# pengsongyou/openscene

Hardware: AMD Instinct MI355X
Metric: active voxels/sec MinkUNet18A fwd+bwd @2cm ScanNet; per-point query ms (higher is better)
Workload: dtype f32 (bf16x6 split-precision MFMA, fp32 accumulate); 1 GPU; ScanNet distillation step (configs[2]): MinkUNet18A, 768-d head, 1 synthetic S100k scene/GPU (100999 voxels on rank 0, 2 cm), training-mode BN; timed = coordinate+kernel maps, forward, cosine loss, backward, gradient all-reduce, Adam step; arch=MinkUNet18A, feature_dim=768, voxels_rank0=100999, parallelism=dp1

## Files before the change

include/openscene_amd.h:

```cpp
#ifndef OPENSCENE_AMD_H
#define OPENSCENE_AMD_H

#include <stddef.h>
#include <stdint.h>

#ifdef __cplusplus
extern "C" {
#endif

#define OSN_OK 0
#define OSN_E_ARG (-1)
#define OSN_E_HIP (-2)
#define OSN_E_WS (-3)
#define OSN_E_RANGE (-4)

typedef void* osn_stream_t;

int osn_version(void);
const char* osn_last_error(void);
int osn_device_ok(void);

int64_t osn_hash_capacity(int64_t n);
size_t osn_coords_unique_ws_bytes(int64_t n);

// ... 138 lines not shown
                         const float* residual, int relu, float momentum, float* mean, float* var,
                         float* running_mean, float* running_var, float* y, void* ws, size_t ws_bytes,
                         osn_stream_t stream);
int osn_bn_backward(const float* x, const float* y, const float* gy, const float* mean,
                    const float* var, const float* gamma, float eps, int relu, int training,
                    float* gx, float* gres, float* ggamma, float* gbeta,
                    int64_t n, int c, void* ws, size_t ws_bytes, osn_stream_t stream);

int osn_bn_apply2(const float* x, const float* mean, const float* var, const float* gamma,
                  const float* beta, float eps, const float* residual, int relu, float* y,
                  float* y2, int64_t ld2, int64_t n, int c, osn_stream_t stream);
int osn_bn_forward_train2(const float* x, int64_t n, int c, const float* gamma, const float* beta, float eps,
                          const float* residual, int relu, float momentum, float* mean, float* var,
                          float* running_mean, float* running_var, float* y, float* y2, int64_t ld2,
                          void* ws, size_t ws_bytes, osn_stream_t stream);
int osn_bn_backward_multi(const float* x, const float* y, const float* const* gy_host, const int64_t* gy_ld_host,
                          int n_gy, const float* mean, const float* var, const float* gamma, float eps, int relu,
                          int training, float* gx, float* gres, float* ggamma, float* gbeta,
                          int64_t n, int c, void* ws, size_t ws_bytes, osn_stream_t stream);
int osn_bn_backward_multi2(const float* x, const float* y, const float* const* gy_host, const int64_t* gy_ld_host, int n_gy,
                           const float* mean, const float* var, const float* gamma, const float* beta, float eps, int relu,
                           int training, float* gx, float* gres, float* ggamma, float* gbeta, int64_t n, int c, void* ws,
                           size_t ws_bytes, osn_stream_t stream);

size_t osn_distill_loss_state_bytes(int64_t n, int64_t n_sel);
int osn_distill_loss_fwd(const float* out, const int64_t* sel, const float* target, int64_t n, int64_t n_sel, int d, int kind,
                         float* loss, void* state, size_t state_bytes, osn_stream_t stream);
int osn_distill_loss_bwd(const float* out, const float* target, const float* gloss, int64_t n, int64_t n_sel, int d, int kind,
                         float* gout, const void* state, size_t state_bytes, osn_stream_t stream);
int osn_distill_loss_bwd_rows(const float* out, const float* target, const float* gloss, int64_t n, int64_t n_sel, int d, int kind,
                              float* gout, float* grows, const void* state, size_t state_bytes, osn_stream_t stream);
int osn_distill_loss_check(const void* state, int64_t n, int64_t n_sel, osn_stream_t stream);

int osn_adam_step(float* params, const float* grads, float* exp_avg, float* exp_avg_sq, int64_t n, int64_t step, float lr,
                  float beta1, float beta2, float eps, float weight_decay, osn_stream_t stream);

int osn_sgd_step(float* params, const float* grads, float* momentum_buf, int64_t n, float lr, float momentum, float dampening,
                 float weight_decay, int nesterov, int first, osn_stream_t stream);

size_t osn_seg_loss_state_bytes(int64_t n_lab, int c);
int osn_seg_loss_fwd(const float* logits, const int64_t* rows, const int64_t* labels, int64_t n, int64_t n_lab, int c,
                     int64_t ignore_index, float* loss, int64_t* pred, int64_t* confusion, void* state, size_t state_bytes,
                     osn_stream_t stream);
int osn_seg_loss_bwd(const float* logits, const int64_t* labels, const float* gloss, int64_t n, int c, int64_t ignore_index,
                     float* glogits, const void* state, size_t state_bytes, osn_stream_t stream);
int osn_seg_loss_check(const void* state, int64_t n, int64_t n_lab, int c, osn_stream_t stream);
// ... 267 lines not shown
```

openscene_amd/_lib.py:

```python
import ctypes
import os
import threading

_HERE = os.path.dirname(os.path.abspath(__file__))
LIB_PATH = os.environ.get("OSN_LIB_PATH") or os.path.join(_HERE, "lib", "libopenscene_amd.so")

_c = ctypes
_vp, _i32, _i64, _sz, _f32 = _c.c_void_p, _c.c_int, _c.c_int64, _c.c_size_t, _c.c_float

PROTOTYPES = {
    "osn_version": (_i32, []),
    "osn_last_error": (_c.c_char_p, []),
    "osn_device_ok": (_i32, []),
    "osn_hash_capacity": (_i64, [_i64]),
    "osn_coords_unique_ws_bytes": (_sz, [_i64]),
    "osn_coords_unique": (_i32, [_vp, _i64, _i32, _vp, _vp, _i64, _vp, _vp, _vp, _c.POINTER(_i64), _vp, _sz, _vp]),
    "osn_coords_unique_async": (_i32, [_vp, _i64, _vp, _i32, _vp, _vp, _i64, _vp, _vp, _vp, _vp, _vp, _vp, _sz, _vp]),
    "osn_coords_pyramid_async": (_i32, [_vp, _i64, _vp, _i32, _vp, _vp, _i64, _vp, _vp, _vp, _vp, _vp, _sz, _vp]),
    "osn_kmap_build": (_i32, [_vp, _vp, _i64, _vp, _i64, _i32, _i32, _vp, _vp, _vp]),
    "osn_kmap_build_self": (_i32, [_vp, _vp, _i64, _vp, _i64, _i32, _i32, _vp, _vp, _vp]),
    "osn_kmap_transpose": (_i32, [_vp, _i64, _i32, _i64, _vp, _vp]),
    "osn_kmap_sort_ws_bytes": (_sz, [_i64]),
    "osn_kmap_sort": (_i32, [_vp, _i64, _i32, _vp, _vp, _vp, _vp, _vp, _sz, _vp]),
    "osn_kmap_count": (_i32, [_vp, _i64, _i32, _vp, _vp]),
# ... 44 lines not shown
    "osn_seg_loss_fwd": (_i32, [_vp, _vp, _vp, _i64, _i64, _i32, _i64, _vp, _vp, _vp, _vp, _sz, _vp]),
    "osn_seg_loss_bwd": (_i32, [_vp, _vp, _vp, _i64, _i32, _i64, _vp, _vp, _sz, _vp]),
    "osn_seg_loss_check": (_i32, [_vp, _i64, _i64, _i32, _vp]),
    "osn_seg_vote": (_i32, [_vp, _vp, _i64, _i64, _i32, _vp, _vp]),
    "osn_spconv_fwd_ws_ws_bytes": (_sz, [_i64, _i32, _i32, _i32]),
    "osn_spconv_fwd_ws": (_i32, [_vp, _i64, _vp, _vp, _i64, _i32, _i32, _vp, _vp, _i64, _i32, _i32, _i32, _vp, _sz, _vp]),
    "osn_spconv_wgrad_tl_partial": (_i32, [_vp, _vp, _vp, _i32, _vp, _i64, _i64, _i32, _i32, _i32, _vp, _sz, _vp, _vp]),
    "osn_wgrad_tl_reduce_batch": (_i32, [_vp, _i32, _vp]),
    "osn_stem_conv_fwd": (_i32, [_vp, _vp, _vp, _vp, _i64, _i32, _i32, _i32, _vp]),
    "osn_bn_ws_bytes": (_sz, [_i64, _i32]),
    "osn_bn_stats": (_i32, [_vp, _i64, _i32, _vp, _vp, _vp, _vp, _f32, _vp, _sz, _vp]),
    "osn_bn_apply": (_i32, [_vp, _vp, _vp, _vp, _vp, _f32, _vp, _i32, _vp, _i64, _i32, _vp]),
    "osn_bn_forward_train": (_i32, [_vp, _i64, _i32, _vp, _vp, _f32, _vp, _i32, _f32, _vp, _vp, _vp, _vp, _vp, _vp, _sz, _vp]),
    "osn_bn_backward": (_i32, [_vp, _vp, _vp, _vp, _vp, _vp, _f32, _i32, _i32, _vp, _vp, _vp, _vp, _i64, _i32,
                               _vp, _sz, _vp]),
    "osn_bn_apply2": (_i32, [_vp, _vp, _vp, _vp, _vp, _f32, _vp, _i32, _vp, _vp, _i64, _i64, _i32, _vp]),
    "osn_spconv_fwd_rg_ok": (_i32, [_i64, _i32, _i32, _i32]),
    "osn_spconv_fwd_rg": (_i32, [_vp, _i64, _vp, _vp, _vp, _vp, _i64, _i32, _i32, _i32, _vp]),
    "osn_bn_forward_train2": (_i32, [_vp, _i64, _i32, _vp, _vp, _f32, _vp, _i32, _f32, _vp, _vp, _vp, _vp, _vp, _vp, _i64, _vp, _sz, _vp]),
    "osn_bn_backward_multi": (_i32, [_vp, _vp, _vp, _vp, _i32, _vp, _vp, _vp, _f32, _i32, _i32, _vp, _vp, _vp, _vp, _i64, _i32,
                                     _vp, _sz, _vp]),
    "osn_bn_backward_multi2": (_i32, [_vp, _vp, _vp, _vp, _i32, _vp, _vp, _vp, _vp, _f32, _i32, _i32, _vp, _vp, _vp, _vp, _i64, _i32,
                                     _vp, _sz, _vp]),
    "osn_net_plan_query": (_i32, [_vp, _vp, _i32, _vp]),
    "osn_net_forward": (_i32, [_vp, _vp, _vp]),
    "osn_net_backward": (_i32, [_vp, _vp, _vp]),
    "osn_maps_build": (_i32, [_vp, _i32, _vp, _i32, _vp, _vp, _vp, _i32, _vp]),
    "osn_events_create": (_vp, [_i32]),
    "osn_events_destroy": (None, [_vp]),
    "osn_prof_create": (_vp, [_i32]),
    "osn_prof_destroy": (None, [_vp]),
    "osn_prof_filter": (_i32, [_vp, _vp, _i32]),
    "osn_prof_read": (_i32, [_vp, _vp, _vp, _i32, _i32]),
    "osn_relu_fwd": (_i32, [_vp, _vp, _i64, _vp]),
    "osn_relu_bwd": (_i32, [_vp, _vp, _vp, _i64, _vp]),
    "osn_add": (_i32, [_vp, _vp, _vp, _i64, _vp]),
    "osn_cat2": (_i32, [_vp, _i32, _vp, _i32, _vp, _i64, _vp]),
    "osn_cat2_bwd": (_i32, [_vp, _vp, _i32, _vp, _i32, _i64, _vp]),
    "osn_cosine_query": (_i32, [_vp, _vp, _vp, _vp, _vp, _i64, _i32, _i32, _vp]),
    "osn_query_ensemble_ws_bytes": (_sz, [_i64]),
    "osn_query_ensemble": (_i32, [_vp, _vp, _vp, _vp, _vp, _vp, _vp, _vp, _i64, _i32, _i32, _vp, _sz, _vp]),
    "osn_cosine_query_vote": (_i32, [_vp, _vp, _vp, _vp, _vp, _i64, _i32, _i32, _vp]),
    "osn_query_ensemble_vote": (_i32, [_vp, _vp, _vp, _vp, _vp, _vp, _vp, _vp, _i64, _i32, _i32, _vp, _sz, _vp]),
    "osn_eval_confusion": (_i32, [_vp, _vp, _i64, _i32, _vp, _vp, _i64, _vp, _i32, _vp, _vp, _i32, _vp]),
    "osn_eval_check": (_i32, [_vp, _vp]),
    "osn_bank_append": (_i32, [_vp, _i64, _vp, _i64, _i32, _vp, _i64, _vp, _vp]),
# ... 99 lines not shown
```

openscene_amd/csrc/bn.hip:

```cpp
#include "common.h"
#include "epilogue.h"

namespace osn {

constexpr int CR_COLS = 64;
constexpr int CR_RL = 16;
constexpr int CR_MAX_BLOCKS = 512;

constexpr int BN_MAX_SRC = 3;
struct GySrc {
    const float* p[BN_MAX_SRC];
    int64_t ld[BN_MAX_SRC];
    int n;
};

__device__ inline float4 gy_load(const GySrc& s, int64_t r, int col) {
    float4 g = *reinterpret_cast<const float4*>(s.p[0] + r * s.ld[0] + col);
#pragma unroll
    for (int i = 1; i < BN_MAX_SRC; ++i)
        if (i < s.n) {
            const float4 v = *reinterpret_cast<const float4*>(s.p[i] + r * s.ld[i] + col);
            g.x += v.x; g.y += v.y; g.z += v.z; g.w += v.w;
        }
    return g;
}


struct ColReducePlan {
    int n_rb;
    int n_cg;
    int rows_per_block;
};

static ColReducePlan plan_colreduce(int64_t n, int c) {
    ColReducePlan p;
    p.n_cg = int(cdiv(c, CR_COLS));
    int64_t rb = cdiv(n, 4 * CR_RL);
    if (rb > CR_MAX_BLOCKS) rb = CR_MAX_BLOCKS;
    if (rb < 1) rb = 1;
    p.rows_per_block = int(cdiv(cdiv(n, rb), CR_RL) * CR_RL);
    p.n_rb = int(cdiv(n, p.rows_per_block));
    if (p.n_rb < 1) p.n_rb = 1;
    return p;
}

template <int MODE, bool STORE_G>
__device__ __forceinline__ void col_reduce_body(const float* __restrict__ x, const float* __restrict__ y, const GySrc gy,
                                                const float* __restrict__ mean, const float* __restrict__ var, float eps,
                                                int relu, int64_t n, int c, int rows_per_block, double* __restrict__ partial,
                                                const float* __restrict__ gamma, const float* __restrict__ beta,
                                                float* __restrict__ gres) {
    static_assert(!STORE_G || MODE == 1, "only the backward sums form g");
    __shared__ double red[2][CR_RL][CR_COLS];
    const int tid = threadIdx.x;
    const int cl = tid & 15, rl = tid >> 4;
    const int col = blockIdx.y * CR_COLS + cl * 4;
    const bool on = col < c;
    const int64_t r0 = int64_t(blockIdx.x) * rows_per_block;
    const int64_t r1 = min(n, r0 + rows_per_block);
    double s1[4] = {0, 0, 0, 0}, s2[4] = {0, 0, 0, 0};
    float4 mu = make_float4(0, 0, 0, 0), is = make_float4(0, 0, 0, 0);
    float4 ga = make_float4(0, 0, 0, 0), be = make_float4(0, 0, 0, 0);
    const bool from_x = MODE == 1 && !STORE_G && relu && !y;
    if (MODE == 1 && on) {
        mu = *reinterpret_cast<const float4*>(mean + col);
        const float4 v = *reinterpret_cast<const float4*>(var + col);
        is = make_float4(bn_is(v.x, eps), bn_is(v.y, eps), bn_is(v.z, eps), bn_is(v.w, eps));
        if (from_x) {
            ga = *reinterpret_cast<const float4*>(gamma + col);
            be = *reinterpret_cast<const float4*>(beta + col);
        }
    }
    if (on) {
        for (int64_t r = r0 + rl; r < r1; r += CR_RL) {
            const float4 xv = *reinterpret_cast<const float4*>(x + r * c + col);
            if (MODE == 0) {
                s1[0] += xv.x; s1[1] += xv.y; s1[2] += xv.z; s1[3] += xv.w;
                s2[0] += double(xv.x) * xv.x; s2[1] += double(xv.y) * xv.y;
                s2[2] += double(xv.z) * xv.z; s2[3] += double(xv.w) * xv.w;
            } else {
                float4 g = gy_load(gy, r, col);
                if (from_x) {
                    g.x = bn_val(xv.x, mu.x, is.x, ga.x, be.x) > 0.f ? g.x : 0.f;
                    g.y = bn_val(xv.y, mu.y, is.y, ga.y, be.y) > 0.f ? g.y : 0.f;
                    g.z = bn_val(xv.z, mu.z, is.z, ga.z, be.z) > 0.f ? g.z : 0.f;
                    g.w = bn_val(xv.w, mu.w, is.w, ga.w, be.w) > 0.f ? g.w : 0.f;
                } else if (relu) {
                    const float4 yv = *reinterpret_cast<const float4*>(y + r * c + col);
                    g.x = yv.x > 0.f ? g.x : 0.f; g.y = yv.y > 0.f ? g.y : 0.f;
                    g.z = yv.z > 0.f ? g.z : 0.f; g.w = yv.w > 0.f ? g.w : 0.f;
                }
                if (STORE_G) *reinterpret_cast<float4*>(gres + r * c + col) = g;
                s1[0] += g.x; s1[1] += g.y; s1[2] += g.z; s1[3] += g.w;
                s2[0] += double(g.x) * ((xv.x - mu.x) * is.x); s2[1] += double(g.y) * ((xv.y - mu.y) * is.y);
                s2[2] += double(g.z) * ((xv.z - mu.z) * is.z); s2[3] += double(g.w) * ((xv.w - mu.w) * is.w);
            }
        }
    }
#pragma unroll
    for (int j = 0; j < 4; ++j) {
        red[0][rl][cl * 4 + j] = s1[j];
        red[1][rl][cl * 4 + j] = s2[j];
    }
    __syncthreads();
    if (tid < 2 * CR_COLS) {
        const int which = tid / CR_COLS, cc = tid % CR_COLS;
        double s = 0;
#pragma unroll
        for (int r = 0; r < CR_RL; ++r) s += red[which][r][cc];
        const int gc = blockIdx.y * CR_COLS + cc;
        if (gc < c) partial[(int64_t(blockIdx.x) * 2 + which) * c + gc] = s;
    }
}

template <int MODE>
__global__ __launch_bounds__(256) void col_reduce_kernel(const float* __restrict__ x, const float* __restrict__ y,
                                                         const GySrc gy, const float* __restrict__ mean,
                                                         const float* __restrict__ var, float eps, int relu, int64_t n,
                                                         int c, int rows_per_block, double* __restrict__ partial,
                                                         const float* __restrict__ gamma, const float* __restrict__ beta) {
    col_reduce_body<MODE, false>(x, y, gy, mean, var, eps, relu, n, c, rows_per_block, partial, gamma, beta, nullptr);
}

__global__ __launch_bounds__(256) void col_reduce_gres_kernel(const float* __restrict__ x, const float* __restrict__ y,
                                                              const GySrc gy, const float* __restrict__ mean,
                                                              const float* __restrict__ var, float eps, int relu, int64_t n,
                                                              int c, int rows_per_block, double* __restrict__ partial,
                                                              float* __restrict__ gres) {
    col_reduce_body<1, true>(x, y, gy, mean, var, eps, relu, n, c, rows_per_block, partial, nullptr, nullptr, gres);
}

constexpr int FIN_COLS = 16, FIN_PARTS = 64;

constexpr int FIN_ITERS = CR_MAX_BLOCKS / FIN_PARTS;

__device__ inline void finalize_sums(const double* __restrict__ partial, int n_rb, int c, double& s1, double& s2,
                                     int& col) {
    __shared__ double red[2][FIN_PARTS][FIN_COLS];
    const int cl = threadIdx.x & (FIN_COLS - 1), part = threadIdx.x / FIN_COLS;
    col = blockIdx.x * FIN_COLS + cl;
    double va[FIN_ITERS], vb[FIN_ITERS];
    const int cc = col < c ? col : 0;
#pragma unroll
    for (int i = 0; i < FIN_ITERS; ++i) {
        const int blk = part + FIN_PARTS * i;
        const int bc = blk < n_rb ? blk : 0;
        va[i] = partial[(int64_t(bc) * 2 + 0) * c + cc];
        vb[i] = partial[(int64_t(bc) * 2 + 1) * c + cc];
    }
    double a = 0, b = 0;
#pragma unroll
    for (int i = 0; i < FIN_ITERS; ++i) {
// ... 33 lines not shown
    double v = s2 / double(n) - m * m;
    if (v < 0) v = 0;
    mean[j] = float(m);
    var[j] = float(v);
    if (running_mean) running_mean[j] = (1.f - momentum) * running_mean[j] + momentum * float(m);
    if (running_var) {
        const double unb = n > 1 ? v * double(n) / double(n - 1) : v;
        running_var[j] = (1.f - momentum) * running_var[j] + momentum * float(unb);
    }
}

__global__ __launch_bounds__(FIN_COLS * FIN_PARTS) void bn_bwd_finalize_kernel(const double* __restrict__ partial,
                                                                              int n_rb, int c,
                                                                              float* __restrict__ sum_g,
                                                                              float* __restrict__ sum_gx) {
    double s1, s2;
    int j;
    finalize_sums(partial, n_rb, c, s1, s2, j);
    if (threadIdx.x >= FIN_COLS || j >= c) return;
    sum_g[j] = float(s1);
    sum_gx[j] = float(s2);
}

__device__ inline float4 ld4(const float* p) { return *reinterpret_cast<const float4*>(p); }


__global__ __launch_bounds__(256) void bn_apply_kernel(const float* __restrict__ x, const float* __restrict__ mean,
                                                       const float* __restrict__ var, const float* __restrict__ gamma,
                                                       const float* __restrict__ beta, float eps,
                                                       const float* __restrict__ residual, int relu,
                                                       float* __restrict__ y, float* __restrict__ y2, int64_t ld2,
                                                       int64_t total4, int c4) {
    for (int64_t e = int64_t(blockIdx.x) * blockDim.x + threadIdx.x; e < total4; e += int64_t(gridDim.x) * blockDim.x) {
        const int col = int(e % c4) * 4;
        const float4 xv = ld4(x + e * 4), mu = ld4(mean + col), vv = ld4(var + col), ga = ld4(gamma + col),
                     be = ld4(beta + col);
        float4 o;
        o.x = bn_val(xv.x, mu.x, bn_is(vv.x, eps), ga.x, be.x);
        o.y = bn_val(xv.y, mu.y, bn_is(vv.y, eps), ga.y, be.y);
        o.z = bn_val(xv.z, mu.z, bn_is(vv.z, eps), ga.z, be.z);
        o.w = bn_val(xv.w, mu.w, bn_is(vv.w, eps), ga.w, be.w);
        if (residual) {
            const float4 rv = ld4(residual + e * 4);
            o.x += rv.x; o.y += rv.y; o.z += rv.z; o.w += rv.w;
        }
        if (relu) {
            o.x = bn_relu(o.x); o.y = bn_relu(o.y); o.z = bn_relu(o.z); o.w = bn_relu(o.w);
        }
        *reinterpret_cast<float4*>(y + e * 4) = o;
        if (y2) *reinterpret_cast<float4*>(y2 + (e / c4) * ld2 + col) = o;
    }
}

template <bool LOAD_G>
__device__ __forceinline__ void bn_bwd_apply_body(const float* __restrict__ x, const float* __restrict__ y, const GySrc& gy,
                                                  const float* __restrict__ mean, const float* __restrict__ var,
                                                  const float* __restrict__ gamma, float eps, int relu, int training,
                                                  const float* __restrict__ sum_g, const float* __restrict__ sum_gx, float inv_n,
                                                  float* __restrict__ gx, float* __restrict__ gres, int64_t total4, int c4,
                                                  const float* __restrict__ beta) {
    const bool from_x = !LOAD_G && relu && !y;
    for (int64_t e = int64_t(blockIdx.x) * blockDim.x + threadIdx.x; e < total4; e += int64_t(gridDim.x) * blockDim.x) {
        const int col = int(e % c4) * 4;
        float4 g = LOAD_G ? ld4(gres + e * 4) : gy_load(gy, e / c4, col);
        const float4 vv = ld4(var + col), ga = ld4(gamma + col);
        const float4 is = make_float4(bn_is(vv.x, eps), bn_is(vv.y, eps), bn_is(vv.z, eps), bn_is(vv.w, eps));
        float4 xv = make_float4(0, 0, 0, 0), mu = make_float4(0, 0, 0, 0);
        if (training || from_x) { xv = ld4(x + e * 4); mu = ld4(mean + col); }
        if (LOAD_G) {
        } else if (from_x) {
            const float4 be = ld4(beta + col);
            g.x = bn_val(xv.x, mu.x, is.x, ga.x, be.x) > 0.f ? g.x : 0.f;
            g.y = bn_val(xv.y, mu.y, is.y, ga.y, be.y) > 0.f ? g.y : 0.f;
            g.z = bn_val(xv.z, mu.z, is.z, ga.z, be.z) > 0.f ? g.z : 0.f;
            g.w = bn_val(xv.w, mu.w, is.w, ga.w, be.w) > 0.f ? g.w : 0.f;
        } else if (relu) {
            const float4 yv = ld4(y + e * 4);
            g.x = yv.x > 0.f ? g.x : 0.f; g.y = yv.y > 0.f ? g.y : 0.f;
            g.z = yv.z > 0.f ? g.z : 0.f; g.w = yv.w > 0.f ? g.w : 0.f;
        }
        if (!LOAD_G && gres) *reinterpret_cast<float4*>(gres + e * 4) = g;
        float4 o;
        if (training) {
            const float4 sg = ld4(sum_g + col), sx = ld4(sum_gx + col);
            o.x = ga.x * is.x * (g.x - sg.x * inv_n - (xv.x - mu.x) * is.x * sx.x * inv_n);
            o.y = ga.y * is.y * (g.y - sg.y * inv_n - (xv.y - mu.y) * is.y * sx.y * inv_n);
            o.z = ga.z * is.z * (g.z - sg.z * inv_n - (xv.z - mu.z) * is.z * sx.z * inv_n);
            o.w = ga.w * is.w * (g.w - sg.w * inv_n - (xv.w - mu.w) * is.w * sx.w * inv_n);
        } else {
            o.x = ga.x * is.x * g.x; o.y = ga.y * is.y * g.y; o.z = ga.z * is.z * g.z; o.w = ga.w * is.w * g.w;
        }
        *reinterpret_cast<float4*>(gx + e * 4) = o;
    }
}

__global__ __launch_bounds__(256) void bn_bwd_apply_kernel(const float* __restrict__ x, const float* __restrict__ y,
                                                           const GySrc gy, const float* __restrict__ mean,
                                                           const float* __restrict__ var, const float* __restrict__ gamma,
                                                           float eps, int relu, int training,
                                                           const float* __restrict__ sum_g,
                                                           const float* __restrict__ sum_gx, float inv_n,
                                                           float* __restrict__ gx, float* __restrict__ gres,
                                                           int64_t total4, int c4, const float* __restrict__ beta) {
    bn_bwd_apply_body<false>(x, y, gy, mean, var, gamma, eps, relu, training, sum_g, sum_gx, inv_n, gx, gres, total4, c4, beta);
}

__global__ __launch_bounds__(256) void bn_bwd_apply_gres_kernel(const float* __restrict__ x, const float* __restrict__ mean,
                                                                const float* __restrict__ var, const float* __restrict__ gamma,
                                                                float eps, int training, const float* __restrict__ sum_g,
                                                                const float* __restrict__ sum_gx, float inv_n,
                                                                float* __restrict__ gx, const float* __restrict__ gres,
                                                                int64_t total4, int c4) {
    bn_bwd_apply_body<true>(x, nullptr, GySrc{}, mean, var, gamma, eps, 0, training, sum_g, sum_gx, inv_n, gx,
                            const_cast<float*>(gres), total4, c4, nullptr);
}

constexpr int SB_THREADS = 1024, SB_RL = 512, SB_PER = 8, SB_COLS = 8;
constexpr int SB_MAX_ROWS = SB_RL * SB_PER;
// ... 86 lines not shown
            const float4 rv = ld4(residual + int64_t(r) * c + col);
            o.x += rv.x; o.y += rv.y; o.z += rv.z; o.w += rv.w;
        }
        if (relu) {
            o.x = bn_relu(o.x); o.y = bn_relu(o.y); o.z = bn_relu(o.z); o.w = bn_relu(o.w);
        }
        *reinterpret_cast<float4*>(y + int64_t(r) * c + col) = o;
        if (y2) *reinterpret_cast<float4*>(y2 + int64_t(r) * ld2 + col) = o;
    }
}

static bool ranges_overlap(const float* a, size_t na, const float* b, size_t nb) {
    const uintptr_t a0 = reinterpret_cast<uintptr_t>(a), b0 = reinterpret_cast<uintptr_t>(b);
    return a0 < b0 + nb * sizeof(float) && b0 < a0 + na * sizeof(float);
}

static int ew_grid(int64_t total4) {
    int64_t g = cdiv(total4, 256);
    if (g > 2048) g = 2048;
    if (g < 1) g = 1;
    return int(g);
}

}

using namespace osn;

extern "C" size_t osn_bn_ws_bytes(int64_t n, int c) {
    (void)n;
    return size_t(CR_MAX_BLOCKS) * 2 * size_t(c) * 8 + 256;
}

extern "C" int osn_bn_stats(const float* x, int64_t n, int c, float* mean, float* var, float* running_mean,
                            float* running_var, float momentum, void* ws, size_t ws_bytes, osn_stream_t stream) {
    hipStream_t st = static_cast<hipStream_t>(stream);
    OSN_REQUIRE(n >= 1 && c >= 4 && (c & 3) == 0, OSN_E_ARG, "osn_bn_stats: need n >= 1 and c %% 4 == 0 (n=%lld c=%d)", (long long)n, c);
    OSN_REQUIRE(x && mean && var && aligned16(x), OSN_E_ARG, "osn_bn_stats: null or unaligned pointer");
    ColReducePlan p = plan_colreduce(n, c);
    const size_t need = size_t(p.n_rb) * 2 * size_t(c) * 8;
    OSN_REQUIRE(ws && ws_bytes >= need, OSN_E_WS, "osn_bn_stats: workspace %zu < %zu", ws_bytes, need);
    double* partial = static_cast<double*>(ws);
    hipLaunchKernelGGL((col_reduce_kernel<0>), dim3(p.n_rb, p.n_cg), dim3(256), 0, st, x, (const float*)nullptr,
                       GySrc{}, (const float*)nullptr, (const float*)nullptr, 0.f, 0, n, c,
                       p.rows_per_block, partial, (const float*)nullptr, (const float*)nullptr);
    hipLaunchKernelGGL(bn_stats_finalize_kernel, dim3(cdiv(c, FIN_COLS)), dim3(FIN_COLS * FIN_PARTS), 0, st, partial, p.n_rb, n, c, mean, var,
                       running_mean, running_var, momentum);
    OSN_LAUNCH_CHECK();
    return OSN_OK;
}

extern "C" int osn_bn_apply2(const float* x, const float* mean, const float* var, const float* gamma, const float* beta,
                             float eps, const float* residual, int relu, float* y, float* y2, int64_t ld2, int64_t n, int c,
                             osn_stream_t stream) {
    hipStream_t st = static_cast<hipStream_t>(stream);
    OSN_REQUIRE(n >= 0 && c >= 4 && (c & 3) == 0, OSN_E_ARG, "osn_bn_apply: need c %% 4 == 0 (c=%d)", c);
    if (n == 0) return OSN_OK;
    OSN_REQUIRE(x && mean && var && gamma && beta && y, OSN_E_ARG, "osn_bn_apply: null pointer");
    OSN_REQUIRE(aligned16(x) && aligned16(y) && aligned16(mean) && aligned16(var) && aligned16(gamma) && aligned16(beta) &&
                    (!residual || aligned16(residual)),
                OSN_E_ARG, "osn_bn_apply: pointers must be 16-byte aligned");
    OSN_REQUIRE(!y2 || (aligned16(y2) && ld2 >= c && (ld2 & 3) == 0), OSN_E_ARG,
                "osn_bn_apply2: the second destination needs a 16-byte aligned pointer and a row stride >= c, %% 4 == 0");
    const int64_t total4 = n * (c / 4);
    hipLaunchKernelGGL(bn_apply_kernel, dim3(ew_grid(total4)), dim3(256), 0, st, x, mean, var, gamma, beta, eps,
                       residual, relu, y, y2, ld2, total4, c / 4);
    OSN_LAUNCH_CHECK();
    return OSN_OK;
}

extern "C" int osn_bn_apply(const float* x, const float* mean, const float* var, const float* gamma, const float* beta,
                            float eps, const float* residual, int relu, float* y, int64_t n, int c,
                            osn_stream_t stream) {
    return osn_bn_apply2(x, mean, var, gamma, beta, eps, residual, relu, y, nullptr, 0, n, c, stream);
}

extern "C" int osn_bn_forward_train2(const float* x, int64_t n, int c, const float* gamma, const float* beta, float eps,
                                     const float* residual, int relu, float momentum, float* mean, float* var,
                                     float* running_mean, float* running_var, float* y, float* y2, int64_t ld2, void* ws,
                                     size_t ws_bytes, osn_stream_t stream) {
    if (n >= 1 && n <= SB_MAX_ROWS && c >= 4 && (c & 3) == 0) {
        hipStream_t st = static_cast<hipStream_t>(stream);
        OSN_REQUIRE(x && mean && var && gamma && beta && y, OSN_E_ARG, "osn_bn_forward_train: null pointer");
        OSN_REQUIRE(aligned16(x) && aligned16(y) && aligned16(gamma) && aligned16(beta) && (!residual || aligned16(residual)),
                    OSN_E_ARG, "osn_bn_forward_train: pointers must be 16-byte aligned");
        OSN_REQUIRE(!y2 || (aligned16(y2) && ld2 >= c && (ld2 & 3) == 0), OSN_E_ARG,
                    "osn_bn_forward_train2: the second destination needs a 16-byte aligned pointer and a row stride >= c, %% 4 == 0");
        hipLaunchKernelGGL(bn_small_fwd_kernel, dim3(unsigned(cdiv(c, SB_COLS))), dim3(SB_THREADS), 0, st, x, int(n), c, gamma,
// ... 28 lines not shown
    OSN_REQUIRE(!beta || aligned16(beta), OSN_E_ARG, "osn_bn_backward: beta must be 16-byte aligned");
    OSN_REQUIRE(aligned16(x) && aligned16(gx) && aligned16(mean) && aligned16(var) && aligned16(gamma) &&
                    aligned16(ggamma) && aligned16(gbeta) && (!y || aligned16(y)) && (!gres || aligned16(gres)),
                OSN_E_ARG, "osn_bn_backward: pointers must be 16-byte aligned");
    GySrc src{};
    src.n = n_gy;
    for (int i = 0; i < BN_MAX_SRC; ++i) {
        const int j = i < n_gy ? i : 0;
        OSN_REQUIRE(gy[j] && aligned16(gy[j]) && gy_ld[j] >= c && (gy_ld[j] & 3) == 0, OSN_E_ARG,
                    "osn_bn_backward: gradient source %d needs a 16-byte aligned pointer and a row stride >= c, %% 4 == 0", j);
        src.p[i] = gy[j];
        src.ld[i] = gy_ld[j];
    }
    ColReducePlan p = plan_colreduce(n, c);
    const size_t need = size_t(p.n_rb) * 2 * size_t(c) * 8;
    OSN_REQUIRE(ws && ws_bytes >= need, OSN_E_WS, "osn_bn_backward: workspace %zu < %zu", ws_bytes, need);
    double* partial = static_cast<double*>(ws);
    const size_t span = size_t(n) * size_t(c);
    bool via_gres = gres != nullptr && !ranges_overlap(gres, span, x, span) && !(y && ranges_overlap(gres, span, y, span)) &&
                    !ranges_overlap(gres, span, gx, span);
    for (int i = 0; via_gres && i < n_gy; ++i)
        via_gres = !ranges_overlap(gres, span, src.p[i], size_t(n - 1) * size_t(src.ld[i]) + size_t(c));
    const dim3 rgrid(p.n_rb, p.n_cg);
    if (via_gres)
        hipLaunchKernelGGL(col_reduce_gres_kernel, rgrid, dim3(256), 0, st, x, y, src, mean, var, eps, relu, n, c,
                           p.rows_per_block, partial, gres);
    else
        hipLaunchKernelGGL((col_reduce_kernel<1>), rgrid, dim3(256), 0, st, x, y, src, mean, var, eps, relu, n, c,
                           p.rows_per_block, partial, gamma, beta);
    hipLaunchKernelGGL(bn_bwd_finalize_kernel, dim3(cdiv(c, FIN_COLS)), dim3(FIN_COLS * FIN_PARTS), 0, st, partial, p.n_rb, c, gbeta, ggamma);
    const int64_t total4 = n * (c / 4);
    if (via_gres)
        hipLaunchKernelGGL(bn_bwd_apply_gres_kernel, dim3(ew_grid(total4)), dim3(256), 0, st, x, mean, var, gamma, eps, training,
                           gbeta, ggamma, 1.f / float(n), gx, (const float*)gres, total4, c / 4);
    else
        hipLaunchKernelGGL(bn_bwd_apply_kernel, dim3(ew_grid(total4)), dim3(256), 0, st, x, y, src, mean, var, gamma, eps,
                           relu, training, gbeta, ggamma, 1.f / float(n), gx, gres, total4, c / 4, beta);
    OSN_LAUNCH_CHECK();
    return OSN_OK;
}

extern "C" int osn_bn_backward_multi(const float* x, const float* y, const float* const* gy, const int64_t* gy_ld, int n_gy,
                                     const float* mean, const float* var, const float* gamma, float eps, int relu,
                                     int training, float* gx, float* gres, float* ggamma, float* gbeta, int64_t n, int c,
                                     void* ws, size_t ws_bytes, osn_stream_t stream) {
    OSN_REQUIRE(!relu || y, OSN_E_ARG, "osn_bn_backward_multi: relu needs y (or osn_bn_backward_multi2 with beta)");
    return osn_bn_backward_multi2(x, y, gy, gy_ld, n_gy, mean, var, gamma, nullptr, eps, relu, training, gx, gres, ggamma, gbeta, n, c,
                                  ws, ws_bytes, stream);
}

extern "C" int osn_bn_backward(const float* x, const float* y, const float* gy, const float* mean, const float* var,
                               const float* gamma, float eps, int relu, int training, float* gx, float* gres,
                               float* ggamma, float* gbeta, int64_t n, int c, void* ws, size_t ws_bytes,
                               osn_stream_t stream) {
    const int64_t ld = c;
    return osn_bn_backward_multi(x, y, &gy, &ld, 1, mean, var, gamma, eps, relu, training, gx, gres, ggamma, gbeta, n, c, ws,
                                 ws_bytes, stream);
}
```

openscene_amd/ops.py:

```python
import ctypes
import os
import threading
import weakref

import torch

from . import _lib
from ._lib import check

_vp = ctypes.c_void_p

_profiler = None


def set_profiler(p):
    global _profiler
    _profiler = p


_raw_stream_of = torch._C._cuda_getCurrentRawStream
_current_device = torch._C._cuda_getDevice


def _prof_start(kind, dev, **meta):
# ... 922 lines not shown
def bn_backward_multi(x, y, gys, mean, var, gamma, eps, relu, training, want_gres, beta=None, gres_out=None):
    dev = x.device
    lib = _prep(dev)
    n, c = x.shape
    if relu and y is None and (beta is None or want_gres):
        raise ValueError("batch-norm backward with ReLU needs y, or beta and no residual")
    views = [_row_view(g, c, "grad_output[%d]" % i) for i, g in enumerate(gys)]
    ptrs = (ctypes.c_void_p * len(views))(*[v[0] for v in views])
    lds = (ctypes.c_int64 * len(views))(*[v[1] for v in views])
    gx = torch.empty_like(x)
    if gres_out is not None and (not want_gres or gres_out.dtype != torch.float32 or gres_out.shape != x.shape or
                                 gres_out.device != dev or not gres_out.is_contiguous()):
        raise ValueError("gres_out must be a contiguous float32 tensor shaped like x, on its device, and needs want_gres")
    gres = (gres_out if gres_out is not None else torch.empty_like(x)) if want_gres else None
    ggamma = torch.empty(c, dtype=torch.float32, device=dev)
    gbeta = torch.empty(c, dtype=torch.float32, device=dev)
    ws = _ws(_cached("osn_bn_ws_bytes", n, c), dev)
    with _Dev(dev):
        check(lib.osn_bn_backward_multi2(_p(x), _p(y), ptrs, lds, len(views), _p(mean), _p(var), _p(gamma),
                                         _p(beta) if (relu and y is None) else None, float(eps),
                                         int(bool(relu)), int(bool(training)), _p(gx), _p(gres), _p(ggamma), _p(gbeta), n, c,
                                         _p(ws), ws.numel(), _stream(dev)), "osn_bn_backward_multi2")
    return gx, gres, ggamma, gbeta


def relu_fwd(x):
    dev = x.device
    lib = _prep(dev)
    x = _f32c(x, "x")
    y = torch.empty_like(x)
    with _Dev(dev):
        check(lib.osn_relu_fwd(_p(x), _p(y), x.numel(), _stream(dev)), "osn_relu_fwd")
    return y


def relu_bwd(y, gy):
    dev = y.device
    lib = _prep(dev)
    gy = _f32c(gy, "grad_output")
    gx = torch.empty_like(y)
    with _Dev(dev):
        check(lib.osn_relu_bwd(_p(y), _p(gy), _p(gx), y.numel(), _stream(dev)), "osn_relu_bwd")
    return gx


def add(a, b):
# ... 1136 lines not shown
```

Measured before the change: 12.44 million voxels/s.

## Keep BN elementwise threads on fixed columns and batch rows in column reductions

The BN column-reduction kernels now load several rows per thread before accumulating (4 for stats, 2 for backward), which gives more memory-level parallelism. The apply and backward-apply kernels get a variant that rounds the grid so the grid-stride keeps each thread on the same channel columns. That variant loads mean, var, gamma and beta once per thread instead of per element and uses pointer increments instead of per-element division. The old flat kernels stay available behind a runtime toggle, and the rounded grid can add up to 127 extra blocks.

```diff
diff --git a/include/openscene_amd.h b/include/openscene_amd.h
--- a/include/openscene_amd.h
+++ b/include/openscene_amd.h
@@ -184,6 +184,9 @@
                            const float* mean, const float* var, const float* gamma, const float* beta, float eps, int relu,
                            int training, float* gx, float* gres, float* ggamma, float* gbeta, int64_t n, int c, void* ws,
                            size_t ws_bytes, osn_stream_t stream);
+
+int osn_bn_apply_plan(int64_t total4, int c4, int* grid, int* flat);
+int osn_bn_set_flat_kernels(int on);
 
 size_t osn_distill_loss_state_bytes(int64_t n, int64_t n_sel);
 int osn_distill_loss_fwd(const float* out, const int64_t* sel, const float* target, int64_t n, int64_t n_sel, int d, int kind,
diff --git a/openscene_amd/_lib.py b/openscene_amd/_lib.py
--- a/openscene_amd/_lib.py
+++ b/openscene_amd/_lib.py
@@ -90,6 +90,8 @@
                                      _vp, _sz, _vp]),
     "osn_bn_backward_multi2": (_i32, [_vp, _vp, _vp, _vp, _i32, _vp, _vp, _vp, _vp, _f32, _i32, _i32, _vp, _vp, _vp, _vp, _i64, _i32,
                                      _vp, _sz, _vp]),
+    "osn_bn_apply_plan": (_i32, [_i64, _i32, _c.POINTER(_i32), _c.POINTER(_i32)]),
+    "osn_bn_set_flat_kernels": (_i32, [_i32]),
     "osn_net_plan_query": (_i32, [_vp, _vp, _i32, _vp]),
     "osn_net_forward": (_i32, [_vp, _vp, _vp]),
     "osn_net_backward": (_i32, [_vp, _vp, _vp]),
diff --git a/openscene_amd/csrc/bn.hip b/openscene_amd/csrc/bn.hip
--- a/openscene_amd/csrc/bn.hip
+++ b/openscene_amd/csrc/bn.hip
@@ -1,5 +1,7 @@
 #include "common.h"
 #include "epilogue.h"
+
+#include <atomic>
 
 namespace osn {
 
@@ -44,13 +46,43 @@
     return p;
 }
 
-template <int MODE, bool STORE_G>
+__device__ inline float4 ld4(const float* p) { return *reinterpret_cast<const float4*>(p); }
+
+#ifndef OSN_BN_ROWS_STATS
+#define OSN_BN_ROWS_STATS 4
+#endif
+#ifndef OSN_BN_ROWS_BWD
+#define OSN_BN_ROWS_BWD 2
+#endif
+#ifndef OSN_BN_ROWS_GRES
+#define OSN_BN_ROWS_GRES 2
+#endif
+
+struct CrRow {
+    float4 x, y, g[BN_MAX_SRC];
+};
+
+template <int MODE>
+__device__ __forceinline__ void cr_load(CrRow& w, const float* __restrict__ x, const float* __restrict__ y, const GySrc& gy,
+                                        bool need_y, int64_t r, int c, int col) {
+    w.x = ld4(x + r * c + col);
+    if (MODE == 1) {
+        w.g[0] = ld4(gy.p[0] + r * gy.ld[0] + col);
+#pragma unroll
+        for (int i = 1; i < BN_MAX_SRC; ++i)
+            if (i < gy.n) w.g[i] = ld4(gy.p[i] + r * gy.ld[i] + col);
+        if (need_y) w.y = ld4(y + r * c + col);
+    }
+}
+
+template <int MODE, bool STORE_G, int R>
 __device__ __forceinline__ void col_reduce_body(const float* __restrict__ x, const float* __restrict__ y, const GySrc gy,
                                                 const float* __restrict__ mean, const float* __restrict__ var, float eps,
                                                 int relu, int64_t n, int c, int rows_per_block, double* __restrict__ partial,
                                                 const float* __restrict__ gamma, const float* __restrict__ beta,
                                                 float* __restrict__ gres) {
     static_assert(!STORE_G || MODE == 1, "only the backward sums form g");
+    static_assert(R >= 1 && R <= 4, "rows in flight");
     __shared__ double red[2][CR_RL][CR_COLS];
     const int tid = threadIdx.x;
     const int cl = tid & 15, rl = tid >> 4;
@@ -62,6 +94,7 @@
     float4 mu = make_float4(0, 0, 0, 0), is = make_float4(0, 0, 0, 0);
     float4 ga = make_float4(0, 0, 0, 0), be = make_float4(0, 0, 0, 0);
     const bool from_x = MODE == 1 && !STORE_G && relu && !y;
+    const bool need_y = MODE == 1 && relu && !from_x;
     if (MODE == 1 && on) {
         mu = *reinterpret_cast<const float4*>(mean + col);
         const float4 v = *reinterpret_cast<const float4*>(var + col);
@@ -71,29 +104,53 @@
             be = *reinterpret_cast<const float4*>(beta + col);
         }
     }
+    auto add_row = [&](const CrRow& w, int64_t r) {
+        const float4 xv = w.x;
+        if (MODE == 0) {
+            s1[0] += xv.x; s1[1] += xv.y; s1[2] += xv.z; s1[3] += xv.w;
+            s2[0] += double(xv.x) * xv.x; s2[1] += double(xv.y) * xv.y;
+            s2[2] += double(xv.z) * xv.z; s2[3] += double(xv.w) * xv.w;
+        } else {
+            float4 g = w.g[0];
+#pragma unroll
+            for (int i = 1; i < BN_MAX_SRC; ++i)
+                if (i < gy.n) { g.x += w.g[i].x; g.y += w.g[i].y; g.z += w.g[i].z; g.w += w.g[i].w; }
+            if (from_x) {
+                g.x = bn_val(xv.x, mu.x, is.x, ga.x, be.x) > 0.f ? g.x : 0.f;
+                g.y = bn_val(xv.y, mu.y, is.y, ga.y, be.y) > 0.f ? g.y : 0.f;
+                g.z = bn_val(xv.z, mu.z, is.z, ga.z, be.z) > 0.f ? g.z : 0.f;
+                g.w = bn_val(xv.w, mu.w, is.w, ga.w, be.w) > 0.f ? g.w : 0.f;
+            } else if (relu) {
+                const float4 yv = w.y;
+                g.x = yv.x > 0.f ? g.x : 0.f; g.y = yv.y > 0.f ? g.y : 0.f;
+                g.z = yv.z > 0.f ? g.z : 0.f; g.w = yv.w > 0.f ? g.w : 0.f;
+            }
+            if (STORE_G) *reinterpret_cast<float4*>(gres + r * c + col) = g;
+            s1[0] += g.x; s1[1] += g.y; s1[2] += g.z; s1[3] += g.w;
+            s2[0] += double(g.x) * ((xv.x - mu.x) * is.x); s2[1] += double(g.y) * ((xv.y - mu.y) * is.y);
+            s2[2] += double(g.z) * ((xv.z - mu.z) * is.z); s2[3] += double(g.w) * ((xv.w - mu.w) * is.w);
+        }
+    };
     if (on) {
-        for (int64_t r = r0 + rl; r < r1; r += CR_RL) {
-            const float4 xv = *reinterpret_cast<const float4*>(x + r * c + col);
-            if (MODE == 0) {
-                s1[0] += xv.x; s1[1] += xv.y; s1[2] += xv.z; s1[3] += xv.w;
-                s2[0] += double(xv.x) * xv.x; s2[1] += double(xv.y) * xv.y;
-                s2[2] += double(xv.z) * xv.z; s2[3] += double(xv.w) * xv.w;
-            } else {
-                float4 g = gy_load(gy, r, col);
-                if (from_x) {
-                    g.x = bn_val(xv.x, mu.x, is.x, ga.x, be.x) > 0.f ? g.x : 0.f;
-                    g.y = bn_val(xv.y, mu.y, is.y, ga.y, be.y) > 0.f ? g.y : 0.f;
-                    g.z = bn_val(xv.z, mu.z, is.z, ga.z, be.z) > 0.f ? g.z : 0.f;
-                    g.w = bn_val(xv.w, mu.w, is.w, ga.w, be.w) > 0.f ? g.w : 0.f;
-                } else if (relu) {
-                    const float4 yv = *reinterpret_cast<const float4*>(y + r * c + col);
-                    g.x = yv.x > 0.f ? g.x : 0.f; g.y = yv.y > 0.f ? g.y : 0.f;
-                    g.z = yv.z > 0.f ? g.z : 0.f; g.w = yv.w > 0.f ? g.w : 0.f;
+        int64_t r = r0 + rl;
+        for (; r + (R - 1) * CR_RL < r1; r += R * CR_RL) {
+            CrRow w[R];
+#pragma unroll
+            for (int k = 0; k < R; ++k) cr_load<MODE>(w[k], x, y, gy, need_y, r + k * CR_RL, c, col);
+#pragma unroll
+            for (int k = 0; k < R; ++k) add_row(w[k], r + k * CR_RL);
+        }
+        if constexpr (R > 1) {
+            if (r < r1) {
+                CrRow w[R - 1];
+#pragma unroll
+                for (int k = 0; k < R - 1; ++k) {
+                    const int64_t rk = r + k * CR_RL;
+                    cr_load<MODE>(w[k], x, y, gy, need_y, rk < r1 ? rk : r, c, col);
                 }
-                if (STORE_G) *reinterpret_cast<float4*>(gres + r * c + col) = g;
-                s1[0] += g.x; s1[1] += g.y; s1[2] += g.z; s1[3] += g.w;
-                s2[0] += double(g.x) * ((xv.x - mu.x) * is.x); s2[1] += double(g.y) * ((xv.y - mu.y) * is.y);
-                s2[2] += double(g.z) * ((xv.z - mu.z) * is.z); s2[3] += double(g.w) * ((xv.w - mu.w) * is.w);
+#pragma unroll
+                for (int k = 0; k < R - 1; ++k)
+                    if (r + k * CR_RL < r1) add_row(w[k], r + k * CR_RL);
             }
         }
     }
@@ -113,21 +170,29 @@
     }
 }
 
+#define OSN_CR_PARAMS                                                                                                          \
+    const float *__restrict__ x, const float *__restrict__ y, const GySrc gy, const float *__restrict__ mean,                    \
+        const float *__restrict__ var, float eps, int relu, int64_t n, int c, int rows_per_block, double *__restrict__ partial
+
 template <int MODE>
-__global__ __launch_bounds__(256) void col_reduce_kernel(const float* __restrict__ x, const float* __restrict__ y,
-                                                         const GySrc gy, const float* __restrict__ mean,
-                                                         const float* __restrict__ var, float eps, int relu, int64_t n,
-                                                         int c, int rows_per_block, double* __restrict__ partial,
-                                                         const float* __restrict__ gamma, const float* __restrict__ beta) {
-    col_reduce_body<MODE, false>(x, y, gy, mean, var, eps, relu, n, c, rows_per_block, partial, gamma, beta, nullptr);
-}
-
-__global__ __launch_bounds__(256) void col_reduce_gres_kernel(const float* __restrict__ x, const float* __restrict__ y,
-                                                              const GySrc gy, const float* __restrict__ mean,
-                                                              const float* __restrict__ var, float eps, int relu, int64_t n,
-                                                              int c, int rows_per_block, double* __restrict__ partial,
-                                                              float* __restrict__ gres) {
-    col_reduce_body<1, true>(x, y, gy, mean, var, eps, relu, n, c, rows_per_block, partial, nullptr, nullptr, gres);
+__global__ __launch_bounds__(256) void col_reduce_kernel(OSN_CR_PARAMS, const float* __restrict__ gamma,
+                                                         const float* __restrict__ beta) {
+    col_reduce_body<MODE, false, MODE == 0 ? OSN_BN_ROWS_STATS : OSN_BN_ROWS_BWD>(x, y, gy, mean, var, eps, relu, n, c, rows_per_block,
+                                                                                  partial, gamma, beta, nullptr);
+}
+
+__global__ __launch_bounds__(256) void col_reduce_gres_kernel(OSN_CR_PARAMS, float* __restrict__ gres) {
+    col_reduce_body<1, true, OSN_BN_ROWS_GRES>(x, y, gy, mean, var, eps, relu, n, c, rows_per_block, partial, nullptr, nullptr, gres);
+}
+
+template <int MODE>
+__global__ __launch_bounds__(256) void col_reduce_1row_kernel(OSN_CR_PARAMS, const float* __restrict__ gamma,
+                                                              const float* __restrict__ beta) {
+    col_reduce_body<MODE, false, 1>(x, y, gy, mean, var, eps, relu, n, c, rows_per_block, partial, gamma, beta, nullptr);
+}
+
+__global__ __launch_bounds__(256) void col_reduce_gres_1row_kernel(OSN_CR_PARAMS, float* __restrict__ gres) {
+    col_reduce_body<1, true, 1>(x, y, gy, mean, var, eps, relu, n, c, rows_per_block, partial, nullptr, nullptr, gres);
 }
 
 constexpr int FIN_COLS = 16, FIN_PARTS = 64;
@@ -207,10 +272,8 @@
     sum_gx[j] = float(s2);
 }
 
-__device__ inline float4 ld4(const float* p) { return *reinterpret_cast<const float4*>(p); }
-
-
-__global__ __launch_bounds__(256) void bn_apply_kernel(const float* __restrict__ x, const float* __restrict__ mean,
+
+__global__ __launch_bounds__(256) void bn_apply_flat_kernel(const float* __restrict__ x, const float* __restrict__ mean,
                                                        const float* __restrict__ var, const float* __restrict__ gamma,
                                                        const float* __restrict__ beta, float eps,
                                                        const float* __restrict__ residual, int relu,
@@ -238,7 +301,7 @@
 }
 
 template <bool LOAD_G>
-__device__ __forceinline__ void bn_bwd_apply_body(const float* __restrict__ x, const float* __restrict__ y, const GySrc& gy,
+__device__ __forceinline__ void bn_bwd_apply_flat_body(const float* __restrict__ x, const float* __restrict__ y, const GySrc& gy,
                                                   const float* __restrict__ mean, const float* __restrict__ var,
                                                   const float* __restrict__ gamma, float eps, int relu, int training,
                                                   const float* __restrict__ sum_g, const float* __restrict__ sum_gx, float inv_n,
@@ -279,6 +342,146 @@
     }
 }
 
+__global__ __launch_bounds__(256) void bn_bwd_apply_flat_kernel(const float* __restrict__ x, const float* __restrict__ y,
+                                                           const GySrc gy, const float* __restrict__ mean,
+                                                           const float* __restrict__ var, const float* __restrict__ gamma,
+                                                           float eps, int relu, int training,
+                                                           const float* __restrict__ sum_g,
+                                                           const float* __restrict__ sum_gx, float inv_n,
+                                                           float* __restrict__ gx, float* __restrict__ gres,
+                                                           int64_t total4, int c4, const float* __restrict__ beta) {
+    bn_bwd_apply_flat_body<false>(x, y, gy, mean, var, gamma, eps, relu, training, sum_g, sum_gx, inv_n, gx, gres, total4, c4, beta);
+}
+
+__global__ __launch_bounds__(256) void bn_bwd_apply_gres_flat_kernel(const float* __restrict__ x, const float* __restrict__ mean,
+                                                                const float* __restrict__ var, const float* __restrict__ gamma,
+                                                                float eps, int training, const float* __restrict__ sum_g,
+                                                                const float* __restrict__ sum_gx, float inv_n,
+                                                                float* __restrict__ gx, const float* __restrict__ gres,
+                                                                int64_t total4, int c4) {
+    bn_bwd_apply_flat_body<true>(x, nullptr, GySrc{}, mean, var, gamma, eps, 0, training, sum_g, sum_gx, inv_n, gx,
+                            const_cast<float*>(gres), total4, c4, nullptr);
+}
+
+__global__ __launch_bounds__(256) void bn_apply_kernel(const float* __restrict__ x, const float* __restrict__ mean,
+                                                       const float* __restrict__ var, const float* __restrict__ gamma,
+                                                       const float* __restrict__ beta, float eps,
+                                                       const float* __restrict__ residual, int relu,
+                                                       float* __restrict__ y, float* __restrict__ y2, int64_t ld2,
+                                                       int64_t total4, int c4) {
+    const unsigned e0 = blockIdx.x * 256u + threadIdx.x, stride = gridDim.x * 256u;
+    if (e0 >= total4) return;
+    const unsigned row0 = e0 / unsigned(c4);
+    const int col = int(e0 - row0 * unsigned(c4)) * 4;
+    const int64_t rstep = stride / unsigned(c4), step = int64_t(stride) * 4;
+    const float4 mu = ld4(mean + col), vv = ld4(var + col), ga = ld4(gamma + col), be = ld4(beta + col);
+    const float4 is = make_float4(bn_is(vv.x, eps), bn_is(vv.y, eps), bn_is(vv.z, eps), bn_is(vv.w, eps));
+    const float* xp = x + int64_t(e0) * 4;
+    const float* rp = residual ? residual + int64_t(e0) * 4 : nullptr;
+    float* yp = y + int64_t(e0) * 4;
+    float* y2p = y2 ? y2 + int64_t(row0) * ld2 + col : nullptr;
+    for (int64_t e = e0; e < total4; e += stride) {
+        const float4 xv = ld4(xp);
+        float4 rv = make_float4(0, 0, 0, 0);
+        if (residual) {
+            rv = ld4(rp);
+            rp += step;
+        }
+        float4 o;
+        o.x = bn_val(xv.x, mu.x, is.x, ga.x, be.x);
+        o.y = bn_val(xv.y, mu.y, is.y, ga.y, be.y);
+        o.z = bn_val(xv.z, mu.z, is.z, ga.z, be.z);
+        o.w = bn_val(xv.w, mu.w, is.w, ga.w, be.w);
+        if (residual) {
+            o.x += rv.x; o.y += rv.y; o.z += rv.z; o.w += rv.w;
+        }
+        if (relu) {
+            o.x = bn_relu(o.x); o.y = bn_relu(o.y); o.z = bn_relu(o.z); o.w = bn_relu(o.w);
+        }
+        *reinterpret_cast<float4*>(yp) = o;
+        if (y2) {
+            *reinterpret_cast<float4*>(y2p) = o;
+            y2p += rstep * ld2;
+        }
+        xp += step;
+        yp += step;
+    }
+}
+
+template <bool LOAD_G>
+__device__ __forceinline__ void bn_bwd_apply_body(const float* __restrict__ x, const float* __restrict__ y, const GySrc& gy,
+                                                  const float* __restrict__ mean, const float* __restrict__ var,
+                                                  const float* __restrict__ gamma, float eps, int relu, int training,
+                                                  const float* __restrict__ sum_g, const float* __restrict__ sum_gx, float inv_n,
+                                                  float* __restrict__ gx, float* __restrict__ gres, int64_t total4, int c4,
+                                                  const float* __restrict__ beta) {
+#pragma clang fp contract(off)
+    const bool from_x = !LOAD_G && relu && !y;
+    const unsigned e0 = blockIdx.x * 256u + threadIdx.x, stride = gridDim.x * 256u;
+    if (e0 >= total4) return;
+    const unsigned row0 = e0 / unsigned(c4);
+    const int col = int(e0 - row0 * unsigned(c4)) * 4;
+    const int64_t rstep = stride / unsigned(c4), step = int64_t(stride) * 4;
+    const float4 z = make_float4(0, 0, 0, 0);
+    const float4 vv = ld4(var + col), ga = ld4(gamma + col);
+    const float4 is = make_float4(bn_is(vv.x, eps), bn_is(vv.y, eps), bn_is(vv.z, eps), bn_is(vv.w, eps));
+    const float4 mu = (training || from_x) ? ld4(mean + col) : z;
+    const float4 be = from_x ? ld4(beta + col) : z;
+    const float4 sg = training ? ld4(sum_g + col) : z, sx = training ? ld4(sum_gx + col) : z;
+    const float4 gi = make_float4(ga.x * is.x, ga.y * is.y, ga.z * is.z, ga.w * is.w);
+    const int64_t off = int64_t(e0) * 4;
+    int64_t so[BN_MAX_SRC], sstep[BN_MAX_SRC];
+#pragma unroll
+    for (int i = 0; i < BN_MAX_SRC; ++i) {
+        so[i] = LOAD_G ? 0 : int64_t(row0) * gy.ld[i] + col;
+        sstep[i] = LOAD_G ? 0 : rstep * gy.ld[i];
+    }
+    for (int64_t e = e0, o4 = off; e < total4; e += stride, o4 += step) {
+        float4 xv = z, yv = z, gs[BN_MAX_SRC];
+        if (training || from_x) xv = ld4(x + o4);
+        if (LOAD_G) {
+            gs[0] = ld4(gres + o4);
+        } else {
+            gs[0] = ld4(gy.p[0] + so[0]);
+            so[0] += sstep[0];
+#pragma unroll
+            for (int i = 1; i < BN_MAX_SRC; ++i)
+                if (i < gy.n) {
+                    gs[i] = ld4(gy.p[i] + so[i]);
+                    so[i] += sstep[i];
+                }
+            if (relu && !from_x) yv = ld4(y + o4);
+        }
+        float4 g = gs[0];
+        if (!LOAD_G) {
+#pragma unroll
+            for (int i = 1; i < BN_MAX_SRC; ++i)
+                if (i < gy.n) { g.x += gs[i].x; g.y += gs[i].y; g.z += gs[i].z; g.w += gs[i].w; }
+        }
+        if (LOAD_G) {
+        } else if (from_x) {
+            g.x = bn_val(xv.x, mu.x, is.x, ga.x, be.x) > 0.f ? g.x : 0.f;
+            g.y = bn_val(xv.y, mu.y, is.y, ga.y, be.y) > 0.f ? g.y : 0.f;
+            g.z = bn_val(xv.z, mu.z, is.z, ga.z, be.z) > 0.f ? g.z : 0.f;
+            g.w = bn_val(xv.w, mu.w, is.w, ga.w, be.w) > 0.f ? g.w : 0.f;
+        } else if (relu) {
+            g.x = yv.x > 0.f ? g.x : 0.f; g.y = yv.y > 0.f ? g.y : 0.f;
+            g.z = yv.z > 0.f ? g.z : 0.f; g.w = yv.w > 0.f ? g.w : 0.f;
+        }
+        if (!LOAD_G && gres) *reinterpret_cast<float4*>(gres + o4) = g;
+        float4 o;
+        if (training) {
+            o.x = gi.x * __fmaf_rn(-((xv.x - mu.x) * is.x * sx.x), inv_n, __fmaf_rn(-sg.x, inv_n, g.x));
+            o.y = gi.y * __fmaf_rn(-((xv.y - mu.y) * is.y * sx.y), inv_n, __fmaf_rn(-sg.y, inv_n, g.y));
+            o.z = gi.z * __fmaf_rn(-((xv.z - mu.z) * is.z * sx.z), inv_n, __fmaf_rn(-sg.z, inv_n, g.z));
+            o.w = gi.w * __fmaf_rn(-((xv.w - mu.w) * is.w * sx.w), inv_n, __fmaf_rn(-sg.w, inv_n, g.w));
+        } else {
+            o.x = gi.x * g.x; o.y = gi.y * g.y; o.z = gi.z * g.z; o.w = gi.w * g.w;
+        }
+        *reinterpret_cast<float4*>(gx + o4) = o;
+    }
+}
+
 __global__ __launch_bounds__(256) void bn_bwd_apply_kernel(const float* __restrict__ x, const float* __restrict__ y,
                                                            const GySrc gy, const float* __restrict__ mean,
                                                            const float* __restrict__ var, const float* __restrict__ gamma,
@@ -411,9 +614,46 @@
     return int(g);
 }
 
+constexpr int EW_SLACK = 127;
+struct ApplyPlan {
+    int grid;
+    bool keep;
+};
+
+static ApplyPlan plan_apply(int64_t total4, int c4) {
+    const int g = ew_grid(total4);
+    int a = c4, b = 256;
+    while (b) { const int t = a % b; a = b; b = t; }
+    const int64_t m = c4 / a;
+    const int64_t up = cdiv(int64_t(g), m) * m;
+    if (up - g <= EW_SLACK) return ApplyPlan{int(up), true};
+    return ApplyPlan{g, false};
+}
+
+static std::atomic<int> g_flat_kernels{0};
+
+#ifndef OSN_BN_KEEP_COLUMNS
+#define OSN_BN_KEEP_COLUMNS 1
+#endif
+
+static ApplyPlan launch_plan_apply(int64_t total4, int c4) {
+    if (!OSN_BN_KEEP_COLUMNS || g_flat_kernels.load(std::memory_order_relaxed)) return ApplyPlan{ew_grid(total4), false};
+    return plan_apply(total4, c4);
+}
+
 }
 
 using namespace osn;
+
+extern "C" int osn_bn_set_flat_kernels(int on) { return g_flat_kernels.exchange(on ? 1 : 0); }
+
+extern "C" int osn_bn_apply_plan(int64_t total4, int c4, int* grid, int* flat) {
+    OSN_REQUIRE(total4 >= 0 && c4 >= 1 && grid && flat, OSN_E_ARG, "osn_bn_apply_plan: need total4 >= 0, c4 >= 1 and two outputs");
+    const ApplyPlan p = plan_apply(total4, c4);
+    *grid = p.grid;
+    *flat = p.keep ? 0 : 1;
+    return OSN_OK;
+}
 
 extern "C" size_t osn_bn_ws_bytes(int64_t n, int c) {
     (void)n;
@@ -429,7 +669,8 @@
     const size_t need = size_t(p.n_rb) * 2 * size_t(c) * 8;
     OSN_REQUIRE(ws && ws_bytes >= need, OSN_E_WS, "osn_bn_stats: workspace %zu < %zu", ws_bytes, need);
     double* partial = static_cast<double*>(ws);
-    hipLaunchKernelGGL((col_reduce_kernel<0>), dim3(p.n_rb, p.n_cg), dim3(256), 0, st, x, (const float*)nullptr,
+    const auto kern = g_flat_kernels.load(std::memory_order_relaxed) ? col_reduce_1row_kernel<0> : col_reduce_kernel<0>;
+    hipLaunchKernelGGL(kern, dim3(p.n_rb, p.n_cg), dim3(256), 0, st, x, (const float*)nullptr,
                        GySrc{}, (const float*)nullptr, (const float*)nullptr, 0.f, 0, n, c,
                        p.rows_per_block, partial, (const float*)nullptr, (const float*)nullptr);
     hipLaunchKernelGGL(bn_stats_finalize_kernel, dim3(cdiv(c, FIN_COLS)), dim3(FIN_COLS * FIN_PARTS), 0, st, partial, p.n_rb, n, c, mean, var,
@@ -451,7 +692,8 @@
     OSN_REQUIRE(!y2 || (aligned16(y2) && ld2 >= c && (ld2 & 3) == 0), OSN_E_ARG,
                 "osn_bn_apply2: the second destination needs a 16-byte aligned pointer and a row stride >= c, %% 4 == 0");
     const int64_t total4 = n * (c / 4);
-    hipLaunchKernelGGL(bn_apply_kernel, dim3(ew_grid(total4)), dim3(256), 0, st, x, mean, var, gamma, beta, eps,
+    const ApplyPlan ap = launch_plan_apply(total4, c / 4);
+    hipLaunchKernelGGL(ap.keep ? bn_apply_kernel : bn_apply_flat_kernel, dim3(ap.grid), dim3(256), 0, st, x, mean, var, gamma, beta, eps,
                        residual, relu, y, y2, ld2, total4, c / 4);
     OSN_LAUNCH_CHECK();
     return OSN_OK;
@@ -526,20 +768,22 @@
     for (int i = 0; via_gres && i < n_gy; ++i)
         via_gres = !ranges_overlap(gres, span, src.p[i], size_t(n - 1) * size_t(src.ld[i]) + size_t(c));
     const dim3 rgrid(p.n_rb, p.n_cg);
+    const bool one_row = g_flat_kernels.load(std::memory_order_relaxed) != 0;
     if (via_gres)
-        hipLaunchKernelGGL(col_reduce_gres_kernel, rgrid, dim3(256), 0, st, x, y, src, mean, var, eps, relu, n, c,
-                           p.rows_per_block, partial, gres);
+        hipLaunchKernelGGL(one_row ? col_reduce_gres_1row_kernel : col_reduce_gres_kernel, rgrid, dim3(256), 0, st, x, y, src, mean,
+                           var, eps, relu, n, c, p.rows_per_block, partial, gres);
     else
-        hipLaunchKernelGGL((col_reduce_kernel<1>), rgrid, dim3(256), 0, st, x, y, src, mean, var, eps, relu, n, c,
-                           p.rows_per_block, partial, gamma, beta);
+        hipLaunchKernelGGL(one_row ? col_reduce_1row_kernel<1> : col_reduce_kernel<1>, rgrid, dim3(256), 0, st, x, y, src, mean, var,
+                           eps, relu, n, c, p.rows_per_block, partial, gamma, beta);
     hipLaunchKernelGGL(bn_bwd_finalize_kernel, dim3(cdiv(c, FIN_COLS)), dim3(FIN_COLS * FIN_PARTS), 0, st, partial, p.n_rb, c, gbeta, ggamma);
     const int64_t total4 = n * (c / 4);
+    const ApplyPlan ap = launch_plan_apply(total4, c / 4);
     if (via_gres)
-        hipLaunchKernelGGL(bn_bwd_apply_gres_kernel, dim3(ew_grid(total4)), dim3(256), 0, st, x, mean, var, gamma, eps, training,
-                           gbeta, ggamma, 1.f / float(n), gx, (const float*)gres, total4, c / 4);
+        hipLaunchKernelGGL(ap.keep ? bn_bwd_apply_gres_kernel : bn_bwd_apply_gres_flat_kernel, dim3(ap.grid), dim3(256), 0, st, x, mean,
+                           var, gamma, eps, training, gbeta, ggamma, 1.f / float(n), gx, (const float*)gres, total4, c / 4);
     else
-        hipLaunchKernelGGL(bn_bwd_apply_kernel, dim3(ew_grid(total4)), dim3(256), 0, st, x, y, src, mean, var, gamma, eps,
-                           relu, training, gbeta, ggamma, 1.f / float(n), gx, gres, total4, c / 4, beta);
+        hipLaunchKernelGGL(ap.keep ? bn_bwd_apply_kernel : bn_bwd_apply_flat_kernel, dim3(ap.grid), dim3(256), 0, st, x, y, src, mean, var,
+                           gamma, eps, relu, training, gbeta, ggamma, 1.f / float(n), gx, gres, total4, c / 4, beta);
     OSN_LAUNCH_CHECK();
     return OSN_OK;
 }
diff --git a/openscene_amd/ops.py b/openscene_amd/ops.py
--- a/openscene_amd/ops.py
+++ b/openscene_amd/ops.py
@@ -968,6 +968,35 @@
                                          int(bool(relu)), int(bool(training)), _p(gx), _p(gres), _p(ggamma), _p(gbeta), n, c,
                                          _p(ws), ws.numel(), _stream(dev)), "osn_bn_backward_multi2")
     return gx, gres, ggamma, gbeta
+
+
+def bn_apply2(x, mean, var, gamma, beta, eps, residual=None, relu=False, y2=None, out=None):
+    dev = x.device
+    lib = _prep(dev)
+    x = _f32c(x, "x")
+    n, c = x.shape
+    if residual is not None:
+        residual = _f32c(residual, "residual")
+        if residual.shape != x.shape:
+            raise ValueError("residual shape %s != %s" % (tuple(residual.shape), tuple(x.shape)))
+    if out is not None and (out.dtype != torch.float32 or out.shape != x.shape or out.device != dev or not out.is_contiguous()):
+        raise ValueError("out must be a contiguous float32 tensor shaped like x, on its device")
+    p2, ld2 = _row_view(y2, c, "y2") if y2 is not None else (None, 0)
+    y = out if out is not None else torch.empty_like(x)
+    with _Dev(dev):
+        check(lib.osn_bn_apply2(_p(x), _p(mean), _p(var), _p(gamma), _p(beta), float(eps), _p(residual), int(bool(relu)),
+                                _p(y), p2, ld2, n, c, _stream(dev)), "osn_bn_apply2")
+    return y
+
+
+def bn_apply_plan(total4, c4):
+    grid, flat = ctypes.c_int32(), ctypes.c_int32()
+    check(_lib.load().osn_bn_apply_plan(int(total4), int(c4), ctypes.byref(grid), ctypes.byref(flat)), "osn_bn_apply_plan")
+    return grid.value, bool(flat.value)
+
+
+def bn_set_flat_kernels(on):
+    return bool(_lib.load().osn_bn_set_flat_kernels(int(bool(on))))
 
 
 def relu_fwd(x):
```

Result: faster. 12.57 million voxels/s (median of 6 runs) (+1.1%).
